# kai-neumann/OrthoSfM

Measured on AMD Instinct MI355X. Metric: image-pairs matched/sec + BA iterations/sec (N images, M tracks) at 1/2/4/8 GPU, higher is better.
Workload: dtype i8; 1 GPU; 50 orthographic images, 20000 SIFT features/img, exhaustive matching (1225 pairs, low-res gate + two-way + cross-check + lists; SURVEY 8d's unit of work: up to, not including, RANSAC-F -- the pass through RANSAC-F is `with_geometric_verification`); views=50, features_per_view=20000, pairs=1225

## Files before the change

include/osfm_hip.h:

```cpp
#ifndef OSFM_HIP_H
#define OSFM_HIP_H

#include <stddef.h>
#include <stdint.h>

#ifdef __cplusplus
extern "C" {
#endif

#define OSFM_API __attribute__((visibility("default")))

typedef enum osfm_status {
    OSFM_OK = 0,
    OSFM_E_ARG = -1,
    OSFM_E_DEVICE = -2,
    OSFM_E_RANGE = -3,
    OSFM_E_CAPACITY = -4,
    OSFM_E_STATE = -5,
    OSFM_E_NUMERIC = -6,
    OSFM_E_IO = -7
} osfm_status;

OSFM_API const char *osfm_last_error(void);
#define OSFM_ABI_VERSION 102
// ... 39 lines not shown
    int32_t min_lowres_matches;
    int32_t min_feature_matches;
    int32_t pairs_per_batch;
    int32_t geometric_verification;
    int32_t ransac_max_iterations;
    double ransac_threshold;
    int32_t min_matching_inliers;
    int32_t matcher_type;
    uint64_t ransac_seed;
    int32_t cascade_keep_empty_blocks;
    int32_t special_kernel_max;
} osfm_match_options;

OSFM_API int osfm_match_options_default(osfm_match_options *opts);

typedef struct osfm_matcher osfm_matcher;

OSFM_API int osfm_match_create(int device, int num_views,
    const osfm_match_options *opts, osfm_matcher **out);
OSFM_API int osfm_match_destroy(osfm_matcher *m);

OSFM_API int osfm_match_create_multi(const int *device_ids, int num_devices, int num_views,
    const osfm_match_options *opts, osfm_matcher **out);
OSFM_API int osfm_match_get_devices(const osfm_matcher *m, int32_t *device_ids, int capacity,
    int32_t *num_devices);

OSFM_API int osfm_quantize_sift(const float *src, int n, uint16_t *dst);
OSFM_API int osfm_quantize_surf(const float *src, int n, int16_t *dst);

OSFM_API int osfm_match_set_view(osfm_matcher *m, int view,
    const uint16_t *sift, int n_sift, const int16_t *surf, int n_surf);
OSFM_API int osfm_match_set_view_float(osfm_matcher *m, int view,
    const float *sift, int n_sift, const float *surf, int n_surf);
OSFM_API int osfm_match_expect_pairs(osfm_matcher *m, int32_t pairs_per_call);
OSFM_API int osfm_match_view_size(const osfm_matcher *m, int view,
    int *n_sift, int *n_surf);

OSFM_API int osfm_match_set_positions(osfm_matcher *m, int view, const float *xy, int n);

OSFM_API int osfm_match_pair(osfm_matcher *m, int view_1, int view_2,
    int32_t *m12, int32_t *len12, int32_t *m21, int32_t *len21);

OSFM_API int osfm_match_pair_lowres(osfm_matcher *m, int view_1, int view_2,
    int num_features, int32_t *count);

OSFM_API int osfm_match_twoway(osfm_matcher *m, int view_1, int view_2,
    int descriptor_type, int num_features, int32_t *m12, int32_t *m21);

typedef struct osfm_pair {
    int32_t view_1;
    int32_t view_2;
} osfm_pair;

enum {
    OSFM_PAIR_MATCHED = 0,
    OSFM_PAIR_REJECTED_LOWRES = 1,
    OSFM_PAIR_REJECTED_COUNT = 2,
    OSFM_PAIR_SKIPPED_EMPTY = 3,
    OSFM_PAIR_REJECTED_INLIERS = 4
};

typedef struct osfm_pair_result {
    int32_t status;
    int32_t lowres_matches;
    int32_t num_matches;
    int32_t num_inliers;
    int64_t offset;
} osfm_pair_result;

OSFM_API int osfm_match_all(osfm_matcher *m, const osfm_pair *pairs,
    int num_pairs, osfm_pair_result *results, int32_t *corr,
    int64_t capacity, int64_t *total);

OSFM_API int osfm_pair_from_index(int64_t index, int32_t *view_1, int32_t *view_2);

typedef struct osfm_match_stats {
    double tile_kernel_ms;
    int32_t tile_kernel_launches;
    int32_t exact_scan_queries;
    int64_t mac_count;
    int64_t algorithmic_bytes;
    double lowres_kernel_ms;
    int32_t lowres_kernel_launches;
    int32_t reserved;
    int64_t lowres_mac_count;
    double cashash_kernel_ms;
    int32_t cashash_kernel_launches;
    int32_t special_kernel_launches;
    double special_kernel_ms;
    double tile_shader_cycles;
    double tile_refclk_ticks;
    double surf_tile_kernel_ms;
    int32_t surf_tile_kernel_launches;
    int32_t reserved2;
    int64_t surf_mac_count;
} osfm_match_stats;
OSFM_API int osfm_match_get_stats(const osfm_matcher *m, osfm_match_stats *out);
OSFM_API int osfm_match_get_shard_stats(const osfm_matcher *m, int shard, osfm_match_stats *out);

OSFM_API int osfm_match_get_cascade_hashes(osfm_matcher *m, int view, int type,
    uint64_t *hashes, uint8_t *bucket_ids);

typedef struct osfm_ransac_options {
    int32_t max_iterations;
    int32_t reserved;
    double threshold;
    uint64_t seed;
} osfm_ransac_options;
OSFM_API int osfm_ransac_options_default(osfm_ransac_options *o);

OSFM_API int osfm_ransac_fundamental(int device, const float *pos1, int n1, const float *pos2, int n2,
    const int32_t *corr, int k, const osfm_ransac_options *opts, uint64_t pair_id,
    int32_t *inliers, int32_t *num_inliers, double *F);


enum {
    OSFM_BA_MODEL_QUATERNION = 0,
    OSFM_BA_MODEL_EULER = 1
};

typedef struct osfm_ba_problem {
    int32_t model;
    int32_t num_cameras;
    int32_t num_points;
    int32_t num_observations;
    double *cam_params;
    const uint8_t *cam_const;
    const int32_t *img_width;
    const int32_t *img_height;
    double *points;
    const double *obs_xy;
    const int32_t *obs_camera;
    const int32_t *obs_point;
} osfm_ba_problem;

typedef struct osfm_ba_options {
    double huber_delta;
    double function_tolerance;
    double gradient_tolerance;
    double parameter_tolerance;
    int32_t max_num_iterations;
    int32_t optimize_points;
    double initial_trust_region_radius;
    double max_trust_region_radius;
    double min_trust_region_radius;
    double min_relative_decrease;
    double min_lm_diagonal;
    double max_lm_diagonal;
    int32_t jacobi_scaling;
    int32_t max_consecutive_invalid_steps;
    int32_t device;
    int32_t verbose;
    int32_t retriangulate_points;
    int32_t reserved;
} osfm_ba_options;

enum {
    OSFM_BA_CONVERGENCE_FUNCTION = 1,
    OSFM_BA_CONVERGENCE_GRADIENT = 2,
    OSFM_BA_CONVERGENCE_PARAMETER = 3,
    OSFM_BA_CONVERGENCE_TRUST_REGION = 4,
    OSFM_BA_NO_CONVERGENCE = 5,
    OSFM_BA_FAILURE = 6
};

typedef struct osfm_ba_summary {
    double initial_cost;
// ... 190 lines not shown
```

orthosfm_amd/capi.py:

```python
from __future__ import annotations

import ctypes as C
import os

import numpy as np

_HERE = os.path.dirname(os.path.abspath(__file__))
LIB_PATH = os.environ.get("OSFM_HIP_LIBRARY") or os.path.join(_HERE, "lib", "libosfm_hip.so")

if not os.path.exists(LIB_PATH):
    raise ImportError(
        f"{LIB_PATH} is missing: build it with `python -c 'import __graft_entry__ as g; g.build()'` "
        "(hipcc --offload-arch=gfx950). orthosfm_amd has no CPU fallback.")

lib = C.CDLL(LIB_PATH)
_hip = C.CDLL("libamdhip64.so")


class OsfmError(RuntimeError):
    def __init__(self, status, msg):
        super().__init__(f"osfm status {status}: {msg}")
        self.status = status


OK, E_ARG, E_DEVICE, E_RANGE, E_CAPACITY, E_STATE, E_NUMERIC, E_IO = 0, -1, -2, -3, -4, -5, -6, -7
MATCHER_EXHAUSTIVE, MATCHER_CASCADE_HASHING = 0, 1
PAIR_MATCHED, PAIR_REJECTED_LOWRES, PAIR_REJECTED_COUNT, PAIR_SKIPPED_EMPTY, PAIR_REJECTED_INLIERS = 0, 1, 2, 3, 4


class MatchOptions(C.Structure):
    _fields_ = [("sift_lowe_ratio", C.c_float), ("sift_distance_threshold", C.c_float),
                ("surf_lowe_ratio", C.c_float), ("surf_distance_threshold", C.c_float),
                ("use_lowres_matching", C.c_int32), ("num_lowres_features", C.c_int32),
                ("min_lowres_matches", C.c_int32), ("min_feature_matches", C.c_int32),
                ("pairs_per_batch", C.c_int32),
                ("geometric_verification", C.c_int32), ("ransac_max_iterations", C.c_int32),
                ("ransac_threshold", C.c_double), ("min_matching_inliers", C.c_int32),
                ("matcher_type", C.c_int32), ("ransac_seed", C.c_uint64),
                ("cascade_keep_empty_blocks", C.c_int32), ("special_kernel_max", C.c_int32)]


class RansacOptions(C.Structure):
    _fields_ = [("max_iterations", C.c_int32), ("reserved", C.c_int32),
                ("threshold", C.c_double), ("seed", C.c_uint64)]


class Pair(C.Structure):
    _fields_ = [("view_1", C.c_int32), ("view_2", C.c_int32)]


class PairResult(C.Structure):
    _fields_ = [("status", C.c_int32), ("lowres_matches", C.c_int32),
                ("num_matches", C.c_int32), ("num_inliers", C.c_int32), ("offset", C.c_int64)]


class MatchStats(C.Structure):
    _fields_ = [("tile_kernel_ms", C.c_double), ("tile_kernel_launches", C.c_int32),
                ("exact_scan_queries", C.c_int32), ("mac_count", C.c_int64),
                ("algorithmic_bytes", C.c_int64), ("lowres_kernel_ms", C.c_double),
                ("lowres_kernel_launches", C.c_int32), ("reserved", C.c_int32),
                ("lowres_mac_count", C.c_int64), ("cashash_kernel_ms", C.c_double),
                ("cashash_kernel_launches", C.c_int32), ("special_kernel_launches", C.c_int32),
                ("special_kernel_ms", C.c_double), ("tile_shader_cycles", C.c_double), ("tile_refclk_ticks", C.c_double),
                ("surf_tile_kernel_ms", C.c_double), ("surf_tile_kernel_launches", C.c_int32), ("reserved2", C.c_int32),
                ("surf_mac_count", C.c_int64)]


class MemoryReport(C.Structure):
    _fields_ = [("device_buffer_bytes", C.c_int64), ("pool_live_bytes", C.c_int64), ("pool_cached_bytes", C.c_int64),
                ("pinned_host_bytes", C.c_int64), ("live_matchers", C.c_int32), ("live_streams", C.c_int32),
                ("live_events", C.c_int32), ("reserved", C.c_int32)]


class BaProblem(C.Structure):
    _fields_ = [("model", C.c_int32), ("num_cameras", C.c_int32), ("num_points", C.c_int32),
                ("num_observations", C.c_int32),
                ("cam_params", C.c_void_p), ("cam_const", C.c_void_p),
                ("img_width", C.c_void_p), ("img_height", C.c_void_p),
                ("points", C.c_void_p), ("obs_xy", C.c_void_p),
                ("obs_camera", C.c_void_p), ("obs_point", C.c_void_p)]


class BaOptions(C.Structure):
    _fields_ = [("huber_delta", C.c_double), ("function_tolerance", C.c_double),
                ("gradient_tolerance", C.c_double), ("parameter_tolerance", C.c_double),
                ("max_num_iterations", C.c_int32), ("optimize_points", C.c_int32),
                ("initial_trust_region_radius", C.c_double), ("max_trust_region_radius", C.c_double),
                ("min_trust_region_radius", C.c_double), ("min_relative_decrease", C.c_double),
                ("min_lm_diagonal", C.c_double), ("max_lm_diagonal", C.c_double),
                ("jacobi_scaling", C.c_int32), ("max_consecutive_invalid_steps", C.c_int32),
                ("device", C.c_int32), ("verbose", C.c_int32),
                ("retriangulate_points", C.c_int32), ("reserved", C.c_int32)]


class TracksSummary(C.Structure):
    _fields_ = [("num_tracks", C.c_int32), ("num_invalid_tracks", C.c_int32), ("num_features", C.c_int64)]


class OutlierStats(C.Structure):
    _fields_ = [("mean", C.c_double), ("sigma", C.c_double),
                ("num_with_point", C.c_int32), ("num_kept", C.c_int32)]


class BaSummary(C.Structure):
    _fields_ = [("initial_cost", C.c_double), ("final_cost", C.c_double),
                ("num_iterations", C.c_int32), ("num_successful_steps", C.c_int32),
                ("num_unsuccessful_steps", C.c_int32), ("termination", C.c_int32),
                ("mean_point_change", C.c_double), ("max_point_change", C.c_double),
                ("solve_ms", C.c_double), ("point_pass_ms", C.c_double),
                ("pair_pass_ms", C.c_double), ("cholesky_ms", C.c_double),
                ("back_pass_ms", C.c_double),
                ("linearizations", C.c_int32), ("num_pair_entries", C.c_int32),
                ("lm_loop_ms", C.c_double),
                ("flow_fallbacks", C.c_int32), ("order_arcs", C.c_int32),
                ("chain_blocks_natural", C.c_int32), ("chain_blocks", C.c_int32)]


class BaLinCapture(C.Structure):
    ARRAYS = ("scale_c", "diag_c", "S", "rhs", "scale_p", "diag_p", "vinv", "ge", "y_c", "cand_cams", "cand_points")
    _fields_ = [(n, C.c_void_p) for n in ARRAYS] + [("nc", C.c_int32), ("reserved", C.c_int32)] + \
               [(n, C.c_double) for n in ("initial_cost", "grad_max", "radius", "model_cost_change", "cand_cost",
                                          "relative_decrease")] + \
               [(n, C.c_int32) for n in ("stopped", "accepted", "flow_aborted", "num_pad")] + \
               [(n, C.c_double) for n in ("pad_diag_min", "pad_diag_max", "pad_off_max")] + \
               [(n, C.c_int32) for n in ("win_num", "win_over", "small_lists", "dense", "dense_splits", "num_pairs", "pair_chunk",
                                         "max_chunks", "multi_chunk_pairs", "order_arcs", "span", "N", "small_solve",
                                         "one_launch", "post_fused", "back_fused")]


EXPORTS = [
    "osfm_last_error", "osfm_version", "osfm_device_count", "osfm_device_memory", "osfm_library_memory", "osfm_trim_device_memory", "osfm_ransac_selfcheck", "osfm_ba_debug_chol_trace", "osfm_ba_debug_flow_spin_limit", "osfm_ba_debug_order",
    "osfm_ba_debug_cholesky_solve", "osfm_ba_debug_linearization",
    "osfm_match_options_default", "osfm_match_create", "osfm_match_create_multi", "osfm_match_get_devices", "osfm_match_destroy",
    "osfm_quantize_sift", "osfm_quantize_surf",
    "osfm_match_set_view", "osfm_match_set_view_float", "osfm_match_view_size", "osfm_match_expect_pairs", "osfm_match_set_positions",
    "osfm_ransac_options_default", "osfm_ransac_fundamental",
    "osfm_match_pair", "osfm_match_pair_lowres", "osfm_match_twoway", "osfm_match_all",
    "osfm_pair_from_index", "osfm_match_get_stats", "osfm_match_get_shard_stats", "osfm_match_get_cascade_hashes",
    "osfm_ba_options_default", "osfm_ba_solve", "osfm_ba_reprojection_errors",
    "osfm_ba_triangulate",
    "osfm_nn_distances", "osfm_filter_outlier_tracks", "osfm_filter_reprojection",
    "osfm_scene_create", "osfm_scene_destroy", "osfm_scene_set_flags", "osfm_scene_align_views", "osfm_scene_set_cameras", "osfm_scene_get_cameras",
    "osfm_scene_triangulate", "osfm_scene_filter_reprojection", "osfm_scene_local_adjustment", "osfm_scene_global_adjustment",
# ... 115 lines not shown
```

orthosfm_amd/csrc/match_api.hip:

```cpp
#include <algorithm>
#include <atomic>
#include <cfloat>
#include <cmath>
#include <cstring>
#include <chrono>
#include <condition_variable>
#include <deque>
#include <functional>
#include <mutex>
#include <queue>
#include <thread>
#include <vector>

#include "match_kernels.h"
#include "cashash_kernels.h"
#include <random>
#include "osfm_common.h"
#include "ransac_kernels.h"

namespace osfm {

static thread_local std::string g_last_error;

void set_error(const char *fmt, ...)
// ... 424 lines not shown
            OSFM_HIP_CHECK(hipEventRecord(m->ev[type][0], s));
            timed[type] = true;
            OSFM_RETURN_IF(m->cas_state.reserve((size_t)std::max<int64_t>(cas_queries[type], 1) * kCasMaxCand * 4));
            launch_cashash_match(type == 0 ? 128 : 64, dp, np, max_n[type], m->cas_state.as<int32_t>(), tab, s);
            OSFM_HIP_CHECK(hipEventRecord(m->ev[type][1], s));
        } else {
            if (total_blocks[type] > 0) { OSFM_HIP_CHECK(hipEventRecord(m->ev[type][0], s)); timed[type] = true; }
            unsigned long long *probe = nullptr;
            if (type == 0 && mode.limit == 0) {
                OSFM_RETURN_IF(m->clock_probe.reserve(16));
                OSFM_HIP_CHECK(hipMemsetAsync(m->clock_probe.ptr, 0, 16, s));
                probe = m->clock_probe.as<unsigned long long>();
                probed = true;
            }
            if (!m->zero_tile.ptr) {
                OSFM_RETURN_IF(m->zero_tile.reserve((size_t)kTileCols * 128));
                OSFM_HIP_CHECK(hipMemsetAsync(m->zero_tile.ptr, 0, (size_t)kTileCols * 128, s));
            }
            launch_match_tiles(type == 0 ? 8 : 4, needs_mask[type], any_special[type], any_c0[type],
                any_corrected[type], dp, np, total_blocks[type],
                m->rowparts.as<RowPart>(), m->colparts.as<ColPart>(), s, probe, m->zero_tile.as<int8_t>());
            if (timed[type]) OSFM_HIP_CHECK(hipEventRecord(m->ev[type][1], s));
            if (type == 0 && !(spjobs.empty() && spjobs_wide.empty())) {
                OSFM_HIP_CHECK(hipEventRecord(m->ev_sp[0], s));
                launch_match_special(dp, m->d_spjobs.as<SpecialJob>(), (int)spjobs.size(), m->sp_parts.as<RowPart>(),
                    m->sp_col.as<int32_t>(), s);
                launch_match_special_wide(dp, m->d_spjobs.as<SpecialJob>() + spjobs.size(), (int)spjobs_wide.size(),
                    m->sp_parts.as<RowPart>(), m->sp_col.as<int32_t>(), s);
                OSFM_HIP_CHECK(hipEventRecord(m->ev_sp[1], s));
            }
            const bool rs = type == 0 && bucketed;
            if (rs) OSFM_HIP_CHECK(hipMemsetAsync(m->rs_count.ptr, 0, (size_t)rs_buckets * sizeof(int32_t), s));
            launch_match_finish(dp, np, max_n[type], m->rowparts.as<RowPart>(),
                m->colparts.as<ColPart>(), m->sp_parts.as<RowPart>(), m->sp_col.as<int32_t>(), tab, 0,
                m->exact_items.as<ExactItem>(), ecount, ecap, rs ? m->rs_count.as<int32_t>() : nullptr,
                rs ? m->rs_items.as<RescoreItem>() : nullptr, s);
            if (rs)
                launch_match_rescore(dp, np, m->rs_count.as<int32_t>(), m->rs_items.as<RescoreItem>(), rs_buckets, tab,
                    m->exact_items.as<ExactItem>(), ecount, ecap, s);
            launch_exact_scan(type == 0 ? 128 : 64, dp, m->exact_items.as<ExactItem>(), ecount, ecap,
                tab, s);
        }
        launch_cross_check_mark(dp, np, max_n[type], m->keep.as<uint8_t>(), m->keep.as<uint8_t>(),
            m->mark_off[type].as<int64_t>(), m->counts[type].as<int32_t>(), s);
        if (mode.apply)
            launch_cross_check_apply(dp, np, max_n[type], m->keep.as<uint8_t>(),
                m->keep.as<uint8_t>(), m->mark_off[type].as<int64_t>(), s);
        OSFM_HIP_CHECK(hipGetLastError());
    }

    std::vector<int32_t> hc[2];
    int32_t hexact[4] = {0, 0, 0, 0};
    for (int type = 0; type < 2; ++type) {
        hc[type].resize(probs[type].size());
        if (!hc[type].empty())
            OSFM_HIP_CHECK(hipMemcpyAsync(hc[type].data(), m->counts[type].ptr,
                hc[type].size() * sizeof(int32_t), hipMemcpyDeviceToHost, s));
    }
    OSFM_HIP_CHECK(hipMemcpyAsync(hexact, m->exact_count.ptr, 16, hipMemcpyDeviceToHost, s));
    unsigned long long hprobe[2] = {0, 0};
    if (probed) OSFM_HIP_CHECK(hipMemcpyAsync(hprobe, m->clock_probe.ptr, 16, hipMemcpyDeviceToHost, s));
    OSFM_HIP_CHECK(hipStreamSynchronize(s));
    m->stats.tile_shader_cycles += (double)hprobe[0];
    m->stats.tile_refclk_ticks += (double)hprobe[1];
    for (int p = 0; p < num_pairs; ++p) {
        int c = 0;
        for (int type = 0; type < 2; ++type)
            if (res->plans[p].prob_index[type] >= 0) c += hc[type][res->plans[p].prob_index[type]];
        res->counts[p] = c;
    }
    for (int type = 0; type < 2; ++type) {
        if (!timed[type]) continue;
        float ms = 0.f;
        OSFM_HIP_CHECK(hipEventElapsedTime(&ms, m->ev[type][0], m->ev[type][1]));
        if (cascade) {
            m->stats.cashash_kernel_ms += ms;
            m->stats.cashash_kernel_launches += 1;
        } else if (mode.limit > 0) {
            m->stats.lowres_kernel_ms += ms;
            m->stats.lowres_kernel_launches += 1;
        } else {
            m->stats.tile_kernel_ms += ms;
            m->stats.tile_kernel_launches += 1;
            if (type == 1) { m->stats.surf_tile_kernel_ms += ms; m->stats.surf_tile_kernel_launches += 1; }
        }
    }
    if (!(spjobs.empty() && spjobs_wide.empty())) {
        float ms = 0.f;
        OSFM_HIP_CHECK(hipEventElapsedTime(&ms, m->ev_sp[0], m->ev_sp[1]));
        m->stats.special_kernel_ms += ms;
        m->stats.special_kernel_launches += 1;
    }
    m->stats.exact_scan_queries += hexact[0] + hexact[1];
    if (cascade) {
    } else if (mode.limit > 0) {
        m->stats.lowres_mac_count += macs;
    } else {
        m->stats.mac_count += macs;
        m->stats.surf_mac_count += macs_surf;
        m->stats.algorithmic_bytes += alg_bytes;
    }
    return OSFM_OK;
}

int upload_view(osfm_matcher *m, int view, const uint16_t *sift, int n_sift, const int16_t *surf,
    int n_surf)
{
    if (view < 0 || view >= (int)m->views.size()) {
        set_error("set_view: view id %d out of range", view);
        return OSFM_E_ARG;
    }
    if (n_sift < 0 || n_surf < 0 || (n_sift > 0 && !sift) || (n_surf > 0 && !surf)) {
        set_error("set_view: null descriptors / negative count");
        return OSFM_E_ARG;
    }
    ViewData &v = m->views[view];
    hipStream_t s = m->up_stream;
    v.set = false;
    v.ns = n_sift; v.nu = n_surf;
    v.ns_pad = round_up(std::max(n_sift, 1), kRowsPerBlock);
    v.nu_pad = round_up(std::max(n_surf, 1), kRowsPerBlock);
    OSFM_RETURN_IF(v.sift.reserve((size_t)v.ns_pad * 128));
    OSFM_RETURN_IF(v.sift_corr.reserve((size_t)v.ns_pad * 4));
    OSFM_RETURN_IF(v.sift_raw.reserve((size_t)v.ns_pad * 128));
    OSFM_RETURN_IF(v.sift_raw_corr.reserve((size_t)v.ns_pad * 4));
    OSFM_RETURN_IF(v.surf.reserve((size_t)v.nu_pad * 64));
    OSFM_RETURN_IF(v.surf_corr.reserve((size_t)v.nu_pad * 4));
    const size_t b_sift = (size_t)n_sift * 128 * 2, b_surf = (size_t)n_surf * 64 * 2;
    const size_t b_ints = (size_t)n_sift * 4 * 2;
    const size_t need = std::max<size_t>(b_sift + b_surf + b_ints, 64);
    const int ps = m->pin_next++ & 1;
    if (m->pin_used[ps]) OSFM_HIP_CHECK(hipEventSynchronize(m->pin_ev[ps]));
    if (m->pin_bytes[ps] < need) {
        pinned_free(m->pin_ptr[ps], m->pin_bytes[ps]);
        m->pin_ptr[ps] = nullptr; m->pin_bytes[ps] = 0;
        OSFM_HIP_CHECK(pinned_alloc(reinterpret_cast<void **>(&m->pin_ptr[ps]), need + need / 4, hipHostMallocDefault));
        m->pin_bytes[ps] = need + need / 4;
    }
    char *pin = m->pin_ptr[ps];
    uint16_t *p_sift = reinterpret_cast<uint16_t *>(pin);
    int16_t *p_surf = reinterpret_cast<int16_t *>(pin + b_sift);
    int32_t *p_special = reinterpret_cast<int32_t *>(pin + b_sift + b_surf), *p_slot = p_special + n_sift;
    int n_special = 0;
    bool bad = false;
    {
        auto rows = [&](int lo, int hi, int *bad_out) {
            int b = 0;
            for (int i = lo; i < hi; ++i) {
                const uint16_t *d = sift + (size_t)i * 128;
                uint16_t *o = p_sift + (size_t)i * 128;
                unsigned mx = 0;
                for (int k = 0; k < 128; ++k) { o[k] = d[k]; mx = std::max<unsigned>(mx, d[k]); }
                b |= mx > 255;
                p_slot[i] = mx > 127 ? 1 : 0;
            }
            *bad_out = b;
        };
        static const int max_thr = getenv("OSFM_UPLOAD_THREADS") ? std::max(1, std::min(4, atoi(getenv("OSFM_UPLOAD_THREADS")))) : 4;
        const int nthr = n_sift >= 8192 ? max_thr : 1;
        int bad_t[4] = {0, 0, 0, 0};
        std::vector<std::thread> th;
        for (int t = 1; t < nthr; ++t)
            th.emplace_back(rows, (int)((int64_t)n_sift * t / nthr), (int)((int64_t)n_sift * (t + 1) / nthr), &bad_t[t]);
        rows(0, (int)((int64_t)n_sift / nthr), &bad_t[0]);
        for (auto &t : th) t.join();
        for (int t = 0; t < nthr; ++t) bad |= bad_t[t] != 0;
// ... 1037 lines not shown
                    chunk_out += h_cnt[jx];
                }
                if (written_out + chunk_out > capacity) overflow = true;
                if (!overflow && chunk_out > 0) {
                    const int ng = (int)g_cnt.size();
                    OSFM_RETURN_IF(m->d_gather_off.reserve((size_t)ng * 20));
                    OSFM_RETURN_IF(m->d_corr2.reserve((size_t)chunk_out * 8));
                    char *gb = m->d_gather_off.as<char>();
                    OSFM_HIP_CHECK(hipMemcpyAsync(gb, g_src.data(), (size_t)ng * 8, hipMemcpyHostToDevice, s));
                    OSFM_HIP_CHECK(hipMemcpyAsync(gb + (size_t)ng * 8, g_dst.data(), (size_t)ng * 8, hipMemcpyHostToDevice, s));
                    OSFM_HIP_CHECK(hipMemcpyAsync(gb + (size_t)ng * 16, g_cnt.data(), (size_t)ng * 4, hipMemcpyHostToDevice, s));
                    launch_gather_inliers(ng, m->d_corr.as<int32_t>(), m->d_inl.as<int32_t>(),
                        reinterpret_cast<const int64_t *>(gb), reinterpret_cast<const int64_t *>(gb + (size_t)ng * 8),
                        reinterpret_cast<const int32_t *>(gb + (size_t)ng * 16), m->d_corr2.as<int32_t>(), s);
                    OSFM_HIP_CHECK(hipGetLastError());
                    OSFM_HIP_CHECK(hipMemcpyAsync(corr + 2 * written_out, m->d_corr2.ptr, (size_t)chunk_out * 8,
                        hipMemcpyDeviceToHost, s));
                    OSFM_HIP_CHECK(hipStreamSynchronize(s));
                    lap("lists on the host");
                }
                written_out += chunk_out;
            }
            written += chunk_corr;
        }
    }
    if (!o.geometric_verification) OSFM_HIP_CHECK(hipStreamSynchronize(m->copy_stream));
    if (o.geometric_verification) written = written_out;
    if (total) *total = written;
    if (overflow) {
        set_error("match_all: %lld correspondences need more than the given capacity %lld",
            (long long)written, (long long)capacity);
        return OSFM_E_CAPACITY;
    }
    return OSFM_OK;
}

}

extern "C" {

int osfm_match_get_cascade_hashes(osfm_matcher *m, int view, int type, uint64_t *hashes,
    uint8_t *bucket_ids)
{
    if (!m || type < 0 || type > 1) { set_error("get_cascade_hashes: bad arguments"); return OSFM_E_ARG; }
    if (!m->shards.empty()) return osfm_match_get_cascade_hashes(m->shards[0], view, type, hashes, bucket_ids);
    std::lock_guard<std::mutex> lock(m->mu);
    OSFM_RETURN_IF(check_view(m, view, "get_cascade_hashes"));
    OSFM_HIP_CHECK(hipSetDevice(m->device));
    OSFM_RETURN_IF(ensure_cashash(m));
    const ViewData &v = m->views[view];
    const int n = type == 0 ? v.ns : v.nu;
    const int words = type == 0 ? 2 : 1;
    if (n > 0 && hashes)
        OSFM_HIP_CHECK(hipMemcpy(hashes, v.cas_hash[type].ptr, (size_t)n * words * 8, hipMemcpyDeviceToHost));
    if (n > 0 && bucket_ids)
        OSFM_HIP_CHECK(hipMemcpy(bucket_ids, v.cas_bucket[type].ptr, (size_t)n * kCasGroups, hipMemcpyDeviceToHost));
    return OSFM_OK;
}

int osfm_match_get_shard_stats(const osfm_matcher *m, int shard, osfm_match_stats *out)
{
    if (!m || !out) { set_error("get_shard_stats: null argument"); return OSFM_E_ARG; }
    const int n = m->shards.empty() ? 1 : (int)m->shards.size();
    if (shard < 0 || shard >= n) { set_error("get_shard_stats: shard %d of %d", shard, n); return OSFM_E_ARG; }
    *out = m->shards.empty() ? m->stats : m->shards[shard]->stats;
    return OSFM_OK;
}

int osfm_match_get_stats(const osfm_matcher *m, osfm_match_stats *out)
{
    if (!m || !out) { set_error("get_stats: null argument"); return OSFM_E_ARG; }
    if (!m->shards.empty()) {
        memset(out, 0, sizeof(*out));
        for (const auto *sh : m->shards) {
            const osfm_match_stats &t = sh->stats;
            out->tile_kernel_ms += t.tile_kernel_ms; out->tile_kernel_launches += t.tile_kernel_launches;
            out->exact_scan_queries += t.exact_scan_queries; out->mac_count += t.mac_count;
            out->algorithmic_bytes += t.algorithmic_bytes; out->lowres_kernel_ms += t.lowres_kernel_ms;
            out->lowres_kernel_launches += t.lowres_kernel_launches; out->lowres_mac_count += t.lowres_mac_count;
            out->cashash_kernel_ms += t.cashash_kernel_ms; out->cashash_kernel_launches += t.cashash_kernel_launches;
            out->special_kernel_launches += t.special_kernel_launches; out->special_kernel_ms += t.special_kernel_ms;
            out->tile_shader_cycles += t.tile_shader_cycles; out->tile_refclk_ticks += t.tile_refclk_ticks;
            out->surf_tile_kernel_ms += t.surf_tile_kernel_ms; out->surf_tile_kernel_launches += t.surf_tile_kernel_launches;
            out->surf_mac_count += t.surf_mac_count;
        }
        return OSFM_OK;
    }
    *out = m->stats;
    return OSFM_OK;
}

}
```

orthosfm_amd/csrc/match_kernels.hip:

```cpp
#include <algorithm>

#include "match_kernels.h"

namespace osfm {


typedef int v4i __attribute__((ext_vector_type(4)));
typedef int v16i __attribute__((ext_vector_type(16)));


__device__ __forceinline__ int max3i(int a, int b, int c)
{
    int r;
    asm("v_max3_i32 %0, %1, %2, %3" : "=v"(r) : "v"(a), "v"(b), "v"(c));
    return r;
}
__device__ __forceinline__ int med3a(int a, int b, int c)
{
    int r;
    asm("v_med3_i32 %0, %1, %2, %3" : "=v"(r) : "v"(a), "v"(b), "v"(c));
    return r;
}

constexpr int kGroupTiles = 8;
// ... 23 lines not shown
template <int CH, bool MASKED, bool RAW, bool C0>
__device__ __forceinline__ void
tile_body(const MatchProblem &pd, int rb, int seg, RowPart *__restrict__ rowparts,
    ColPart *__restrict__ colparts, char *smem, const int8_t *__restrict__ zero_tile)
{
    static_assert(!C0 || RAW, "the correction-free form needs the raw row operand");
    constexpr int D = CH * 16;
    constexpr int KS = CH / 2;
    constexpr int RPB = 16 / CH;
    constexpr int TILE_BYTES = kTileCols * D;
    constexpr int CHUNKS = kTileCols * CH;
    constexpr int CPT = CHUNKS / 256;
    constexpr int BBUF_BYTES = 2 * TILE_BYTES > 16384 ? 2 * TILE_BYTES : 16384;
    constexpr int kRawShift = C0 ? kPipeTileBits : 7;
    constexpr int kCurNone = RAW ? -(1 << (30 - kRawShift)) : kKeyNone;
    static_assert(kSegCols / kTileCols <= (1 << 7), "tile index must fit the key");
    constexpr bool PIPE = C0;
    constexpr int NCHUNK = 2 * KS;
    constexpr int RPC = 16 / NCHUNK;
    constexpr int CPC = 16 / KS;

    char *bbuf = smem;
    int *corrbuf = reinterpret_cast<int *>(smem + BBUF_BYTES);
    ColPart *colbuf = reinterpret_cast<ColPart *>(smem + BBUF_BYTES + 2 * 64 * 4);
    int *rsecbuf = reinterpret_cast<int *>(smem + BBUF_BYTES + 2 * 64 * 4 + 8 * 4 * 64 * 8);

    const int n1 = pd.n1, n2 = pd.n2, n2stride = pd.n2stride;
    const int8_t *const Bbase = C0 ? pd.B_raw : pd.B;
    const int32_t *const corrBbase = pd.corrB;
    int32_t *const colbest = reinterpret_cast<int32_t *>(colparts + pd.colpart_off) + (int64_t)rb * pd.n2stride;
    int32_t *const colsecond = colbest + (int64_t)pd.nrb * pd.n2stride;
    const int tid = threadIdx.x;
    const int wave = tid >> 6, lane = tid & 63, lr = lane & 31, lh = lane >> 5;
    const int row0 = rb * kRowsPerBlock + wave * 64;
    const int gcode = wave * 2 + lh;

    const int8_t *Abase = pd.A;
    const int32_t *corrA = pd.corrA;
    int arow0 = row0;
    if (RAW) { Abase = pd.A_raw; corrA = pd.corrA_raw; }
    else if (!MASKED && rb >= pd.nrb_main) {
        Abase = pd.A_special; corrA = pd.corrA_special;
        arow0 = (rb - pd.nrb_main) * kRowsPerBlock + wave * 64;
    }
    v4i a[2][KS];
    v16i ra[2];
#pragma unroll
    for (int rf = 0; rf < 2; ++rf) {
        const int8_t *arow = Abase + (size_t)(arow0 + rf * 32 + lr) * D;
#pragma unroll
        for (int ks = 0; ks < KS; ++ks)
            a[rf][ks] = *reinterpret_cast<const v4i *>(arow + (ks * 2 + lh) * 16);
#pragma unroll
        for (int r = 0; r < 16; ++r)
            ra[rf][r] = C0 ? 0 : corrA[arow0 + rf * 32 + (r & 3) + 8 * (r >> 2) + 4 * lh];
    }
    const v16i zero16 = {0, 0, 0, 0, 0, 0, 0, 0, 0, 0, 0, 0, 0, 0, 0, 0};
    unsigned row_valid_bits = 0xffffffffu;
    if (MASKED) {
        row_valid_bits = 0;
#pragma unroll
        for (int fr = 0; fr < 32; ++fr) {
            const int row = row0 + (fr >> 4) * 32 + (fr & 3) + 8 * ((fr >> 2) & 3) + 4 * lh;
            row_valid_bits |= (row < n1 ? 1u : 0u) << fr;
        }
    }

    v16i rbest[2], rcur[2];
#pragma unroll
    for (int rf = 0; rf < 2; ++rf)
#pragma unroll
        for (int r = 0; r < 16; ++r) {
            rbest[rf][r] = kKeyNone; rcur[rf][r] = kCurNone;
            rsecbuf[(rf * 16 + r) * 256 + tid] = kKeyNone;
        }

    const int seg_cols = pd.seg_cols;
    const int col_begin = seg * seg_cols;
    const int col_lim = min(n2, col_begin + seg_cols);
    const int ntiles = (col_lim - col_begin + kTileCols - 1) / kTileCols;

    typedef __attribute__((address_space(3))) void lds_void;
    typedef const __attribute__((address_space(1))) void glb_void;
    const int wave_s = __builtin_amdgcn_readfirstlane(wave);
    unsigned lane4 = (unsigned)lane * 4u;
    if (PIPE) asm volatile("" : "+v"(lane4));
    unsigned lane_off[CPT];
#pragma unroll
    for (int c = 0; c < CPT; ++c) {
        const int q = (c * 4 + wave) * 64 + lane;
        const int col = q / CH;
        const int ch = (q % CH) ^ ((col / RPB) % CH);
        lane_off[c] = (unsigned)(col * D + ch * 16);
    }
    auto dma_wait = [&](bool store_behind = false) {
        if (!PIPE) return;
#ifndef OSFM_TILE_WAIT_ALL
        if (store_behind) { asm volatile("s_waitcnt vmcnt(2)" ::: "memory"); return; }
#endif
        asm volatile("s_waitcnt vmcnt(0)" ::: "memory");
    };
    auto stage_tile = [&](int t, int buf) {
        const int8_t *src = Bbase + (size_t)(col_begin + t * kTileCols) * D;
        if (PIPE && t >= ntiles) src = zero_tile;
#pragma unroll
        for (int c = 0; c < CPT; ++c) {
            const int q0 = (c * 4 + wave_s) * 64;
            if (PIPE) {
                static_assert(!PIPE || RAW, "the PIPE schedule must not contain compiler-managed m0 users");
                const unsigned lds_at = (unsigned)(uintptr_t)(bbuf + buf * TILE_BYTES + q0 * 16);
                asm volatile("s_mov_b32 m0, %2\n\tglobal_load_lds_dwordx4 %0, %1"
                             :: "v"(lane_off[c]), "s"(src), "s"(lds_at) : "memory");
            } else {
                __builtin_amdgcn_global_load_lds(
                    (glb_void *)(src + lane_off[c]),
                    (lds_void *)(uintptr_t)(bbuf + buf * TILE_BYTES + q0 * 16), 16, 0, 0);
            }
        }
        if (!RAW && wave_s == 0)
            __builtin_amdgcn_global_load_lds(
                (glb_void *)(corrBbase + col_begin + t * kTileCols + lane),
                (lds_void *)(uintptr_t)(corrbuf + buf * 64), 4, 0, 0);
    };

    v4i b[2][KS];
    int cb_next[2] = {0, 0};
    auto load_b = [&](int buf, int cf) {
        const int col = cf * 32 + lr;
        const int swz = (col / RPB) % CH;
#pragma unroll
        for (int ks = 0; ks < KS; ++ks)
            b[cf][ks] = *reinterpret_cast<const v4i *>(
                bbuf + buf * TILE_BYTES + col * D + (((ks * 2 + lh) ^ swz) * 16));
        if (!RAW) cb_next[cf] = corrbuf[buf * 64 + col];
    };

    int cbj[2] = {0, 0}, cjt[2] = {0, 0};
    bool col_valid[2] = {true, true};
    int g[2] = {kValNone, kValNone};

    v16i acc0[2], acc1[2];

    auto phase = [&](auto ph_c, auto cl_c, auto mg_c, auto rs_c, v16i (&cur)[2], v16i (&nxt)[2], int buf_next,
                     int tile0, int tm, int tms) {
        constexpr int PH = decltype(ph_c)::value;
        constexpr int CL = decltype(cl_c)::value;
        constexpr int RS = decltype(rs_c)::value;
        constexpr bool MG = decltype(mg_c)::value != 0;
        constexpr int OF = PH ^ 1;
        int sv = 0;
        ColPart cpm[4];
        if (CL >= 0) sv = rsecbuf[(OF * 16 + CL) * 256 + tid];
        if (MG) {
#pragma unroll
            for (int w = 0; w < 4; ++w) cpm[w] = colbuf[((tm & 7) * 4 + w) * 64 + lane];
        }
#pragma unroll
        for (int i = 0; i < NCHUNK; ++i) {
            const int cf = i / KS, ks = i % KS;
            if (ks == 0)
                nxt[cf] = __builtin_amdgcn_mfma_i32_32x32x32_i8(a[PH ^ 1][0], b[cf][0], C0 ? zero16 : ra[PH ^ 1], 0, 0, 0);
            else
                nxt[cf] = __builtin_amdgcn_mfma_i32_32x32x32_i8(a[PH ^ 1][ks], b[cf][ks], nxt[cf], 0, 0, 0);
            if (PH == 0 && i == KS - 1) load_b(buf_next, 0);
            if (PH == 1 && i == 0) {
                __builtin_amdgcn_sched_barrier(0);
                load_b(buf_next, 1);
            }

#pragma unroll
            for (int r = i * RPC; r < (i + 1) * RPC; ++r) {
                if (RAW) {
                    if (RS >= 0 && r == RS) rcur[PH][r] = max(cur[0][r], cur[1][r]);
                    else rcur[PH][r] = max(max(rcur[PH][r], cur[0][r]), cur[1][r]);
                } else {
                    int k0 = (int)(((unsigned)cur[0][r] << 8) + (unsigned)cjt[0]);
                    int k1 = (int)(((unsigned)cur[1][r] << 8) + (unsigned)cjt[1]);
                    if (MASKED) {
                        k0 = col_valid[0] ? k0 : kKeyNone;
                        k1 = col_valid[1] ? k1 : kKeyNone;
                    }
                    rcur[PH][r] = max3i(rcur[PH][r], k0, k1);
                }
            }
            {
                int x[CPC];
#pragma unroll
                for (int j = 0; j < CPC; ++j) {
                    x[j] = cur[cf][ks * CPC + j];
                    if (MASKED) x[j] = ((row_valid_bits >> (PH * 16 + ks * CPC + j)) & 1u) ? x[j] : kValNone;
                }
                int gg;
                if (PH == 0 && ks == 0) gg = max(x[0], x[1]);
                else gg = max(max(g[cf], x[0]), x[1]);
#pragma unroll
                for (int j = 2; j < CPC; j += 2) gg = max(max(gg, x[j]), x[j + 1]);
                asm volatile("" : "+v"(gg));
                g[cf] = gg;
            }
            if (CL >= 0 && i == 2) {
                const int r = CL;
                const int gk = (int)(((unsigned)rcur[OF][r] << kRawShift) | (unsigned)tile0);
                rsecbuf[(OF * 16 + r) * 256 + tid] = med3a(rbest[OF][r], sv, gk);
                rbest[OF][r] = max(rbest[OF][r], gk);
            }
            if (MG && (i == 2 || i == 3)) {
                if (i == 2) {
                    int k1 = cpm[0].key_best, k2 = cpm[0].key_second;
#pragma unroll
                    for (int w = 1; w < 4; ++w) {
                        k2 = max(max(min(k1, cpm[w].key_best), k2), cpm[w].key_second);
                        k1 = max(k1, cpm[w].key_best);
                    }
                    cpm[0].key_best = k1; cpm[0].key_second = k2;
                } else {
                    store_colpart_sbase(colbest + col_begin + tms * kTileCols, colsecond + col_begin + tms * kTileCols, lane4, cpm[0]);
                }
            }
            __builtin_amdgcn_sched_barrier(0);
        }
    };

    stage_tile(0, 0);
    stage_tile(PIPE || ntiles > 1 ? 1 : 0, 1);
    dma_wait();
    __syncthreads();
    load_b(0, 0);
    load_b(0, 1);
#pragma unroll
    for (int cf = 0; cf < 2; ++cf) {
        acc0[cf] = __builtin_amdgcn_mfma_i32_32x32x32_i8(a[0][0], b[cf][0], C0 ? zero16 : ra[0], 0, 0, 0);
#pragma unroll
        for (int ks = 1; ks < KS; ++ks)
            acc0[cf] = __builtin_amdgcn_mfma_i32_32x32x32_i8(a[0][ks], b[cf][ks], acc0[cf], 0, 0, 0);
    }
    __syncthreads();

    auto tile_top = [&](int t) {
        stage_tile(PIPE ? t + 2 : min(t + 2, ntiles - 1), t & 1);
#pragma unroll
        for (int cf = 0; cf < 2; ++cf) {
            if (!RAW) {
                cbj[cf] = cb_next[cf];
                cjt[cf] = (int)(((unsigned)cbj[cf] << 8) + (unsigned)(t * 2 + cf));
                asm volatile("" : "+v"(cjt[cf]));
            }
            col_valid[cf] = (col_begin + t * kTileCols + cf * 32 + lr) < n2;
        }
    };
    auto tile_bottom = [&](int t, bool store_behind = false) {
        int kk[2];
#pragma unroll
        for (int cf = 0; cf < 2; ++cf) {
            kk[cf] = (int)((unsigned)(g[cf] + cbj[cf]) << 8) | gcode;
            if (MASKED) kk[cf] = g[cf] < -(1 << 27) ? kKeyNone : kk[cf];
        }
        const auto sw = __builtin_amdgcn_permlane32_swap((unsigned)kk[0], (unsigned)kk[1], false, false);
        const int x0 = (int)sw[0], x1 = (int)sw[1];
        ColPart cp;
        cp.key_best = max(x0, x1);
        cp.key_second = min(x0, x1);
        colbuf[((t & 7) * 4 + wave) * 64 + lane] = cp;
        dma_wait(store_behind);
        __syncthreads();
    };
    auto close_all = [&](auto first_tile) {
        int sv[2][16];
#pragma unroll
        for (int rf = 0; rf < 2; ++rf)
#pragma unroll
            for (int r = 0; r < 16; ++r) sv[rf][r] = rsecbuf[(rf * 16 + r) * 256 + tid];
#pragma unroll
        for (int rf = 0; rf < 2; ++rf)
#pragma unroll
            for (int r = 0; r < 16; ++r) {
                const int gk = RAW ? (int)(((unsigned)rcur[rf][r] << kRawShift) | (unsigned)first_tile(rf, r)) : rcur[rf][r];
                rsecbuf[(rf * 16 + r) * 256 + tid] = med3a(rbest[rf][r], sv[rf][r], gk);
                rbest[rf][r] = max(rbest[rf][r], gk);
                rcur[rf][r] = kCurNone;
            }
    };
    auto merge_tile = [&](int tm) {
        ColPart cp[4];
#pragma unroll
        for (int w = 0; w < 4; ++w) cp[w] = colbuf[((tm & 7) * 4 + w) * 64 + lane];
        int k1 = cp[0].key_best, k2 = cp[0].key_second;
#pragma unroll
        for (int w = 1; w < 4; ++w) {
            k2 = max(max(min(k1, cp[w].key_best), k2), cp[w].key_second);
            k1 = max(k1, cp[w].key_best);
        }
        const int col = col_begin + tm * kTileCols + lane;
        if (col < n2stride) {
            ColPart out;
            out.key_best = k1;
            out.key_second = k2;
            store_colpart(colbest, colsecond, (unsigned)col * 4u, out);
        }
    };

    int t = 0;
    if (PIPE) {
        static_assert(kPipeGroupTiles == 16, "the staggered schedule closes one of 16 slots per phase");
        auto cycle_tile = [&](auto u_c, int t0) {
            constexpr int u = decltype(u_c)::value;
            const int tt = t0 + u;
            tile_top(tt);
            const int bn = (tt & 1) ^ 1;
            const int tm = max(tt - 5, 0) + wave;
            phase(IntC<0>(), IntC<u>(), IntC<(u & 3) == 1 ? 1 : 0>(), IntC<(u + 15) & 15>(), acc0, acc1, bn,
                max(tt - 16, 0), tm, max(tt - 5, 0) + wave_s);
            phase(IntC<1>(), IntC<u>(), IntC<0>(), IntC<u>(), acc1, acc0, bn, max(tt - 15, 0), 0, 0);
            tile_bottom(tt, (u & 3) == 1);
        };
        const int tcyc = (ntiles + 15) & ~15;
        for (; t < tcyc; t += 16) {
            cycle_tile(IntC<0>(), t); cycle_tile(IntC<1>(), t); cycle_tile(IntC<2>(), t); cycle_tile(IntC<3>(), t);
            cycle_tile(IntC<4>(), t); cycle_tile(IntC<5>(), t); cycle_tile(IntC<6>(), t); cycle_tile(IntC<7>(), t);
            cycle_tile(IntC<8>(), t); cycle_tile(IntC<9>(), t); cycle_tile(IntC<10>(), t); cycle_tile(IntC<11>(), t);
            cycle_tile(IntC<12>(), t); cycle_tile(IntC<13>(), t); cycle_tile(IntC<14>(), t); cycle_tile(IntC<15>(), t);
        }
        merge_tile(t - 4 + wave);
        rcur[0][15] = kCurNone;
        const int tc = t;
        close_all([&](int rf, int r) { return max(tc - (rf ? 16 : 15) + r, 0); });
    }
    const int t_tail = t;
    if (!PIPE)
    for (; t < ntiles; ++t) {
        tile_top(t);
        phase(IntC<0>(), IntC<-1>(), IntC<0>(), IntC<-1>(), acc0, acc1, (t & 1) ^ 1, 0, 0, 0);
        phase(IntC<1>(), IntC<-1>(), IntC<0>(), IntC<-1>(), acc1, acc0, (t & 1) ^ 1, 0, 0, 0);
        if (PIPE ? t == ntiles - 1 : ((t % kGroupTiles) == kGroupTiles - 1 || t == ntiles - 1)) {
            const int first = PIPE ? t_tail : (t / kGroupTiles) * kGroupTiles;
            close_all([&](int, int) { return first; });
        }
        tile_bottom(t);
        if ((t & 3) == 3 || t == ntiles - 1) {
            const int tm = (t & ~3) + wave;
            if (tm <= t) merge_tile(tm);
        }
    }

    RowPart *rp = rowparts + pd.rowpart_off + (int64_t)seg * ((int64_t)pd.nrb * kRowsPerBlock);
    int *bb = reinterpret_cast<int *>(smem);
    static_assert(BBUF_BYTES + 2 * 64 * 4 + 8 * 4 * 64 * 8 >= 32 * 256 * 4, "the best keys of both fragments must fit in front of rsecbuf");
    __syncthreads();
#pragma unroll
    for (int rf = 0; rf < 2; ++rf)
#pragma unroll
        for (int r = 0; r < 16; ++r) bb[(rf * 16 + r) * 256 + tid] = rbest[rf][r];
    __syncthreads();
    {
        constexpr int SH = RAW ? kRawShift : 8;
        const int r = lane & 15, h = (lane >> 4) & 1, rf = lane >> 5;
        const int base = (rf * 16 + r) * 256 + wave * 64 + h * 32;
        v4i kb[8], ks[8];
#pragma unroll
        for (int j = 0; j < 8; ++j) {
            const int jj = (j + r) & 7;
            kb[j] = *reinterpret_cast<const v4i *>(bb + base + jj * 4);
            ks[j] = *reinterpret_cast<const v4i *>(rsecbuf + base + jj * 4);
        }
        int b1 = kKeyNone, b2 = kKeyNone, smax = kKeyNone;
#pragma unroll
        for (int j = 0; j < 8; ++j)
#pragma unroll
            for (int e = 0; e < 4; ++e) {
                b2 = med3a(b1, b2, kb[j][e]);
                b1 = max(b1, kb[j][e]);
            }
#pragma unroll
        for (int j = 0; j < 8; j += 2)
#pragma unroll
            for (int e = 0; e < 4; ++e) smax = max3i(smax, ks[j][e], ks[j + 1][e]);
        unsigned hit = 0;
#pragma unroll
        for (int j = 7; j >= 0; --j)
#pragma unroll
            for (int e = 3; e >= 0; --e) hit = (hit << 1) | (kb[j][e] == b1 ? 1u : 0u);
        const unsigned rot = __builtin_amdgcn_alignbit(hit, hit, (32 - 4 * r) & 31);
        const int bl = 31 - __builtin_clz(rot | 1u);
        const int sk = max(b2, smax);
        const int row = row0 + rf * 32 + (r & 3) + 8 * (r >> 2) + 4 * h;
        RowPart out;
        out.ip_best = b1 == kKeyNone ? INT_MIN : (b1 >> SH);
        out.ip_second = sk == kKeyNone ? INT_MIN : (sk >> SH);
        out.idx_best = b1 == kKeyNone ? 0
                     : RAW ? col_begin + (b1 & ((1 << kRawShift) - 1)) * kTileCols + bl
                           : col_begin + (b1 & 255) * 32 + bl;
        out.pad = RAW ? 1 : 0;
        rp[row] = out;
    }
}

template <int CH, bool MASKED, bool RAW, bool C0>
__global__ __launch_bounds__(256, 2) void
match_tile_kernel(const MatchProblem *__restrict__ problems, int num_problems, int total_blocks,
    RowPart *__restrict__ rowparts, ColPart *__restrict__ colparts, unsigned long long *__restrict__ clock_probe,
    const int8_t *__restrict__ zero_tile)
{
    extern __shared__ __attribute__((aligned(16))) char smem[];
    const int lin = xcd_remap(blockIdx.x, total_blocks);
    int lo = 0, hi = num_problems - 1;
    while (lo < hi) {
        const int mid = (lo + hi + 1) >> 1;
        if (problems[mid].block_start <= lin) lo = mid; else hi = mid - 1;
    }
    const MatchProblem &pd = problems[lo];
    const int local = lin - pd.block_start;
    const int rb = local / pd.nseg;
    const int seg = local - rb * pd.nseg;
    if (!MASKED && (rb < pd.nrb_main) != RAW) return;
    if (RAW && (pd.c0 != 0) != C0) return;
    if (C0 && clock_probe != nullptr && (blockIdx.x & 1023) == 0) {
// ... 896 lines not shown
```

Measured before the change: 23250 pairs/s.

## Pre-issue first MFMA across barrier, prefetch tile source, and stop pipeline at exact tile count

After: 23490 pairs/s, median of 6. 1.0% higher.

```diff
diff --git a/include/osfm_hip.h b/include/osfm_hip.h
--- a/include/osfm_hip.h
+++ b/include/osfm_hip.h
@@ -145,7 +145,7 @@
     int64_t algorithmic_bytes;
     double lowres_kernel_ms;
     int32_t lowres_kernel_launches;
-    int32_t reserved;
+    int32_t tile_workgroups;
     int64_t lowres_mac_count;
     double cashash_kernel_ms;
     int32_t cashash_kernel_launches;
diff --git a/orthosfm_amd/capi.py b/orthosfm_amd/capi.py
--- a/orthosfm_amd/capi.py
+++ b/orthosfm_amd/capi.py
@@ -58,7 +58,7 @@
     _fields_ = [("tile_kernel_ms", C.c_double), ("tile_kernel_launches", C.c_int32),
                 ("exact_scan_queries", C.c_int32), ("mac_count", C.c_int64),
                 ("algorithmic_bytes", C.c_int64), ("lowres_kernel_ms", C.c_double),
-                ("lowres_kernel_launches", C.c_int32), ("reserved", C.c_int32),
+                ("lowres_kernel_launches", C.c_int32), ("tile_workgroups", C.c_int32),
                 ("lowres_mac_count", C.c_int64), ("cashash_kernel_ms", C.c_double),
                 ("cashash_kernel_launches", C.c_int32), ("special_kernel_launches", C.c_int32),
                 ("special_kernel_ms", C.c_double), ("tile_shader_cycles", C.c_double), ("tile_refclk_ticks", C.c_double),
diff --git a/orthosfm_amd/csrc/match_api.hip b/orthosfm_amd/csrc/match_api.hip
--- a/orthosfm_amd/csrc/match_api.hip
+++ b/orthosfm_amd/csrc/match_api.hip
@@ -530,6 +530,7 @@
         } else {
             m->stats.tile_kernel_ms += ms;
             m->stats.tile_kernel_launches += 1;
+            m->stats.tile_workgroups += total_blocks[type];
             if (type == 1) { m->stats.surf_tile_kernel_ms += ms; m->stats.surf_tile_kernel_launches += 1; }
         }
     }
@@ -1733,7 +1734,7 @@
             out->special_kernel_launches += t.special_kernel_launches; out->special_kernel_ms += t.special_kernel_ms;
             out->tile_shader_cycles += t.tile_shader_cycles; out->tile_refclk_ticks += t.tile_refclk_ticks;
             out->surf_tile_kernel_ms += t.surf_tile_kernel_ms; out->surf_tile_kernel_launches += t.surf_tile_kernel_launches;
-            out->surf_mac_count += t.surf_mac_count;
+            out->surf_mac_count += t.surf_mac_count; out->tile_workgroups += t.tile_workgroups;
         }
         return OSFM_OK;
     }
diff --git a/orthosfm_amd/csrc/match_kernels.hip b/orthosfm_amd/csrc/match_kernels.hip
--- a/orthosfm_amd/csrc/match_kernels.hip
+++ b/orthosfm_amd/csrc/match_kernels.hip
@@ -129,7 +129,8 @@
 
     typedef __attribute__((address_space(3))) void lds_void;
     typedef const __attribute__((address_space(1))) void glb_void;
-    const int wave_s = __builtin_amdgcn_readfirstlane(wave);
+    int wave_s = __builtin_amdgcn_readfirstlane(wave);
+    if (PIPE) asm volatile("" : "+s"(wave_s));
     unsigned lane4 = (unsigned)lane * 4u;
     if (PIPE) asm volatile("" : "+v"(lane4));
     unsigned lane_off[CPT];
@@ -147,9 +148,12 @@
 #endif
         asm volatile("s_waitcnt vmcnt(0)" ::: "memory");
     };
-    auto stage_tile = [&](int t, int buf) {
+    auto tile_src = [&](int t) {
         const int8_t *src = Bbase + (size_t)(col_begin + t * kTileCols) * D;
         if (PIPE && t >= ntiles) src = zero_tile;
+        return src;
+    };
+    auto stage_tile_at = [&](const int8_t *src, int t, int buf) {
 #pragma unroll
         for (int c = 0; c < CPT; ++c) {
             const int q0 = (c * 4 + wave_s) * 64;
@@ -169,6 +173,8 @@
                 (glb_void *)(corrBbase + col_begin + t * kTileCols + lane),
                 (lds_void *)(uintptr_t)(corrbuf + buf * 64), 4, 0, 0);
     };
+    auto stage_tile = [&](int t, int buf) { stage_tile_at(tile_src(t), t, buf); };
+    const int8_t *pf_src = nullptr;
 
     v4i b[2][KS];
     int cb_next[2] = {0, 0};
@@ -188,9 +194,10 @@
 
     v16i acc0[2], acc1[2];
 
-    auto phase = [&](auto ph_c, auto cl_c, auto mg_c, auto rs_c, v16i (&cur)[2], v16i (&nxt)[2], int buf_next,
+    auto phase = [&](auto ph_c, auto cl_c, auto mg_c, auto rs_c, auto pre_c, v16i (&cur)[2], v16i (&nxt)[2], int buf_next,
                      int tile0, int tm, int tms) {
         constexpr int PH = decltype(ph_c)::value;
+        constexpr bool PRE = decltype(pre_c)::value != 0;
         constexpr int CL = decltype(cl_c)::value;
         constexpr int RS = decltype(rs_c)::value;
         constexpr bool MG = decltype(mg_c)::value != 0;
@@ -205,7 +212,9 @@
 #pragma unroll
         for (int i = 0; i < NCHUNK; ++i) {
             const int cf = i / KS, ks = i % KS;
-            if (ks == 0)
+            if (PRE && i == 0)
+                ;
+            else if (ks == 0)
                 nxt[cf] = __builtin_amdgcn_mfma_i32_32x32x32_i8(a[PH ^ 1][0], b[cf][0], C0 ? zero16 : ra[PH ^ 1], 0, 0, 0);
             else
                 nxt[cf] = __builtin_amdgcn_mfma_i32_32x32x32_i8(a[PH ^ 1][ks], b[cf][ks], nxt[cf], 0, 0, 0);
@@ -249,7 +258,9 @@
                 const int r = CL;
                 const int gk = (int)(((unsigned)rcur[OF][r] << kRawShift) | (unsigned)tile0);
                 rsecbuf[(OF * 16 + r) * 256 + tid] = med3a(rbest[OF][r], sv, gk);
-                rbest[OF][r] = max(rbest[OF][r], gk);
+                int nb = max(rbest[OF][r], gk);
+                if (PIPE) asm volatile("" : "+v"(nb));
+                rbest[OF][r] = nb;
             }
             if (MG && (i == 2 || i == 3)) {
                 if (i == 2) {
@@ -268,6 +279,11 @@
         }
     };
 
+    auto first_mfma = [&]() {
+        acc1[0] = __builtin_amdgcn_mfma_i32_32x32x32_i8(a[1][0], b[0][0], C0 ? zero16 : ra[1], 0, 0, 0);
+        __builtin_amdgcn_sched_barrier(0);
+    };
+
     stage_tile(0, 0);
     stage_tile(PIPE || ntiles > 1 ? 1 : 0, 1);
     dma_wait();
@@ -281,10 +297,21 @@
         for (int ks = 1; ks < KS; ++ks)
             acc0[cf] = __builtin_amdgcn_mfma_i32_32x32x32_i8(a[0][ks], b[cf][ks], acc0[cf], 0, 0, 0);
     }
+    if (PIPE) {
+        first_mfma();
+        pf_src = tile_src(2);
+        asm volatile("" : "+s"(pf_src));
+    }
     __syncthreads();
 
     auto tile_top = [&](int t) {
-        stage_tile(PIPE ? t + 2 : min(t + 2, ntiles - 1), t & 1);
+        if (PIPE) {
+            stage_tile_at(pf_src, t + 2, t & 1);
+            pf_src = tile_src(t + 3);
+            asm volatile("" : "+s"(pf_src));
+        } else {
+            stage_tile(min(t + 2, ntiles - 1), t & 1);
+        }
 #pragma unroll
         for (int cf = 0; cf < 2; ++cf) {
             if (!RAW) {
@@ -295,7 +322,7 @@
             col_valid[cf] = (col_begin + t * kTileCols + cf * 32 + lr) < n2;
         }
     };
-    auto tile_bottom = [&](int t, bool store_behind = false) {
+    auto tile_bottom = [&](int t, bool store_behind = false, bool pre_issue = false) {
         int kk[2];
 #pragma unroll
         for (int cf = 0; cf < 2; ++cf) {
@@ -308,6 +335,7 @@
         cp.key_best = max(x0, x1);
         cp.key_second = min(x0, x1);
         colbuf[((t & 7) * 4 + wave) * 64 + lane] = cp;
+        if (pre_issue) first_mfma();
         dma_wait(store_behind);
         __syncthreads();
     };
@@ -354,30 +382,57 @@
             const int tt = t0 + u;
             tile_top(tt);
             const int bn = (tt & 1) ^ 1;
-            const int tm = max(tt - 5, 0) + wave;
-            phase(IntC<0>(), IntC<u>(), IntC<(u & 3) == 1 ? 1 : 0>(), IntC<(u + 15) & 15>(), acc0, acc1, bn,
-                max(tt - 16, 0), tm, max(tt - 5, 0) + wave_s);
-            phase(IntC<1>(), IntC<u>(), IntC<0>(), IntC<u>(), acc1, acc0, bn, max(tt - 15, 0), 0, 0);
-            tile_bottom(tt, (u & 3) == 1);
+            const int tm0 = u >= 5 ? tt - 5 : max(tt - 5, 0);
+            const int tm = tm0 + wave;
+            phase(IntC<0>(), IntC<u>(), IntC<(u & 3) == 1 ? 1 : 0>(), IntC<(u + 15) & 15>(), IntC<1>(), acc0, acc1, bn,
+                max(tt - 16, 0), tm, tm0 + wave_s);
+            phase(IntC<1>(), IntC<u>(), IntC<0>(), IntC<u>(), IntC<0>(), acc1, acc0, bn, max(tt - 15, 0), 0, 0);
+            tile_bottom(tt, (u & 3) == 1, true);
+            return tt + 1 >= ntiles;
         };
-        const int tcyc = (ntiles + 15) & ~15;
-        for (; t < tcyc; t += 16) {
+        for (; t + 16 < ntiles; t += 16) {
             cycle_tile(IntC<0>(), t); cycle_tile(IntC<1>(), t); cycle_tile(IntC<2>(), t); cycle_tile(IntC<3>(), t);
             cycle_tile(IntC<4>(), t); cycle_tile(IntC<5>(), t); cycle_tile(IntC<6>(), t); cycle_tile(IntC<7>(), t);
             cycle_tile(IntC<8>(), t); cycle_tile(IntC<9>(), t); cycle_tile(IntC<10>(), t); cycle_tile(IntC<11>(), t);
             cycle_tile(IntC<12>(), t); cycle_tile(IntC<13>(), t); cycle_tile(IntC<14>(), t); cycle_tile(IntC<15>(), t);
         }
-        merge_tile(t - 4 + wave);
-        rcur[0][15] = kCurNone;
-        const int tc = t;
-        close_all([&](int rf, int r) { return max(tc - (rf ? 16 : 15) + r, 0); });
+        do {
+            if (cycle_tile(IntC<0>(), t)) break;
+            if (cycle_tile(IntC<1>(), t)) break;
+            if (cycle_tile(IntC<2>(), t)) break;
+            if (cycle_tile(IntC<3>(), t)) break;
+            if (cycle_tile(IntC<4>(), t)) break;
+            if (cycle_tile(IntC<5>(), t)) break;
+            if (cycle_tile(IntC<6>(), t)) break;
+            if (cycle_tile(IntC<7>(), t)) break;
+            if (cycle_tile(IntC<8>(), t)) break;
+            if (cycle_tile(IntC<9>(), t)) break;
+            if (cycle_tile(IntC<10>(), t)) break;
+            if (cycle_tile(IntC<11>(), t)) break;
+            if (cycle_tile(IntC<12>(), t)) break;
+            if (cycle_tile(IntC<13>(), t)) break;
+            if (cycle_tile(IntC<14>(), t)) break;
+            cycle_tile(IntC<15>(), t);
+        } while (false);
+        const int tl = ntiles - 1, ue = tl & 15, t0 = tl & ~15;
+        const int tf = max((tl - 1) & ~3, 0);
+        if (tf + wave_s <= tl) merge_tile(tf + wave_s);
+        if (tf + 4 + wave_s <= tl) merge_tile(tf + 4 + wave_s);
+#pragma unroll
+        for (int r = 0; r < 16; ++r) rcur[0][r] = r == ue ? kCurNone : rcur[0][r];
+        close_all([&](int rf, int r) {
+            if (rf) return r <= ue ? t0 + r : max(t0 - 16 + r, 0);
+            return r < ue ? t0 + r + 1 : r > ue ? max(t0 - 15 + r, 0) : 0;
+        });
+        t = ntiles;
+        dma_wait();
     }
     const int t_tail = t;
     if (!PIPE)
     for (; t < ntiles; ++t) {
         tile_top(t);
-        phase(IntC<0>(), IntC<-1>(), IntC<0>(), IntC<-1>(), acc0, acc1, (t & 1) ^ 1, 0, 0, 0);
-        phase(IntC<1>(), IntC<-1>(), IntC<0>(), IntC<-1>(), acc1, acc0, (t & 1) ^ 1, 0, 0, 0);
+        phase(IntC<0>(), IntC<-1>(), IntC<0>(), IntC<-1>(), IntC<0>(), acc0, acc1, (t & 1) ^ 1, 0, 0, 0);
+        phase(IntC<1>(), IntC<-1>(), IntC<0>(), IntC<-1>(), IntC<0>(), acc1, acc0, (t & 1) ^ 1, 0, 0, 0);
         if (PIPE ? t == ntiles - 1 : ((t % kGroupTiles) == kGroupTiles - 1 || t == ntiles - 1)) {
             const int first = PIPE ? t_tail : (t / kGroupTiles) * kGroupTiles;
             close_all([&](int, int) { return first; });
```
